# monoamine11231/Example-GUI-OpenCL-Raytracer

Hardware: AMD Instinct MI355X
Metric: Mrays/s at 1920x1080 depth 4, aggregate over n_gpus; rays = path segments + shadow rays as the reference casts them (value_traced: only those the kernel really traces) (higher is better)
Workload: dtype f32; 1 GPU; C2: scenes/render.map (regenerated), camera raypng.c:17-21, 1920x1080, depth 4, 2 soft-shadow samples, 4x256^2 textures + 4096x3072 skybox (procedural); frame=1920x1080, arithmetic=fast

## Files before the change

example_gui_opencl_raytracer_amd/csrc/hip_wrap.cpp:

```cpp
#include <hip/hip_runtime.h>

#include <algorithm>
#include <cstdarg>
#include <cstdint>
#include <cstdio>
#include <cstdlib>
#include <cmath>
#include <cstring>
#include <string>
#include <vector>

#include "../../include/hip_wrap_ext.h"
#include "png_codec.h"
#include "scene_prep.h"
#include "whitted_params.h"

extern "C" hipError_t wt_fast_launch_trace(const whitted_params*, int, unsigned, size_t, hipStream_t);
extern "C" hipError_t wt_fast_launch_raygen(const raygen_params*, hipStream_t);
extern "C" hipError_t wt_strict_launch_trace(const whitted_params*, int, unsigned, size_t, hipStream_t);
extern "C" hipError_t wt_strict_launch_raygen(const raygen_params*, hipStream_t);
extern "C" hipError_t wt_fast_launch_unit(int, const float*, float*, unsigned, unsigned, unsigned, unsigned, hipStream_t);
extern "C" hipError_t wt_strict_launch_unit(int, const float*, float*, unsigned, unsigned, unsigned, unsigned, hipStream_t);
extern "C" hipError_t wt_fast_launch_unit_scene(const whitted_params*, int, int, const float*, float*, unsigned, unsigned, unsigned, size_t, hipStream_t);
extern "C" hipError_t wt_strict_launch_unit_scene(const whitted_params*, int, int, const float*, float*, unsigned, unsigned, unsigned, size_t, hipStream_t);
// ... 77 lines not shown
    ArgValue values[__MAX_BUFFERS];
};

struct TimingEntry { hipEvent_t start, stop; cl_uint kernel; };

struct Impl {
    int device = 0;
    hipStream_t own_stream = nullptr;
    hipStream_t stream = nullptr;
    std::vector<Kernel> kernels;
    std::vector<Buffer*> live;
    int depth = 15;
    int strict = 0;
    int fuse = 1;
    int async = 0;
    int variant = 0;
    int last_trace_flags = -1;
    int counting = 0;
    float through = 0.8f;
    int stamps = 0;
    uint64_t id_offset = 0;
    uint32_t band_stride = 1, band_phase = 0;
    int supersample = 1;
    float* debug_rgb = nullptr;
    std::vector<clw_sample_camera> cams;
    float aperture = 0.0f, focus = 1.0f;
    std::vector<clw_sample_camera> cams_used;
    float* d_cams = nullptr;
    wt_cam_table cams_dev{}; bool cams_dev_valid = false;
    hipEvent_t cams_fence = nullptr; bool cams_fence_pending = false, cams_in_flight = false;
    const Buffer *prep_s = nullptr, *prep_p = nullptr, *prep_l = nullptr;
    uint32_t prep_ns = 0, prep_np = 0, prep_nl = 0;
    float* d_geom = nullptr; size_t geom_f4 = 0;
    float* d_ptex = nullptr;
    bool have_lpt = false;
    uint64_t scene_generation = 0;
    uint32_t *d_grid_start = nullptr, *d_grid_items = nullptr, *d_grid_box = nullptr;
    float* d_grid_geom = nullptr;
    wprep_grid grid{}; bool grid_ok = false, grid_pair = false; int use_grid = 1;
    unsigned long long* d_counters = nullptr;
    int sched = 1;
    struct Sched {
        unsigned* cost[2] = {nullptr, nullptr}; unsigned* order[2] = {nullptr, nullptr};
        hipEvent_t built[2] = {nullptr, nullptr};
        bool have[2] = {false, false};
        int wr = 0;
        hipEvent_t traced = nullptr;
        uint32_t w = 0, rows = 0, cap = 0;
        int ss = 1;
        wt_cam_table sig_cams{}; bool sig_has_cams = false;
        RaygenArgs sig{}; int sig_depth = 0; uint64_t sig_scene = 0; bool sig_valid = false; int sig_age = 0, newest = 0; uint64_t frame = 0, newest_frame = 0;
        void reset() { have[0] = have[1] = false; sig_valid = false; newest = 0; }
        void free_all() {
            for (int i = 0; i < 2; i++) {
                if (cost[i]) (void)hipFree(cost[i]);
                if (order[i]) (void)hipFree(order[i]);
                if (built[i]) (void)hipEventDestroy(built[i]);
                cost[i] = order[i] = nullptr; built[i] = nullptr;
            }
            if (traced) { (void)hipEventDestroy(traced); traced = nullptr; }
            reset();
        }
    };
    hipStream_t sched_stream = nullptr;
    static constexpr int MAX_CHUNKS = 4;
    Sched scheds[1 + MAX_CHUNKS];
// ... 173 lines not shown
float env_float(const char* name, float dflt) {
    const char* s = getenv(name);
    if (!s || !*s) return dflt;
    char* end = nullptr;
    const float v = strtof(s, &end);
    return (end == s || *end) ? NAN : v;
}

void xorshift_jump_matrices(uint32_t steps, uint32_t out[7][32]) {
    auto apply = [](const uint32_t* A, uint32_t x) { uint32_t r = 0; for (int b = 0; b < 32; b++) if ((x >> b) & 1u) r ^= A[b]; return r; };
    auto mul = [&](const uint32_t* A, const uint32_t* B, uint32_t* C) { uint32_t t[32]; for (int b = 0; b < 32; b++) t[b] = apply(A, B[b]); memcpy(C, t, sizeof t); };
    uint32_t T[32], R[32], Bp[32];
    for (int b = 0; b < 32; b++) { uint32_t x = 1u << b; x ^= x << 13; x ^= x >> 17; x ^= x << 5; T[b] = x; R[b] = 1u << b; }
    memcpy(Bp, T, sizeof T);
    for (uint32_t e = steps; e; e >>= 1) { if (e & 1u) mul(Bp, R, R); mul(Bp, Bp, Bp); }
    memcpy(out[0], R, sizeof R);
    for (int i = 1; i < 7; i++) mul(out[i - 1], out[i - 1], out[i]);
}

void prepare_scene(Impl* I, Buffer* s, uint32_t ns, Buffer* p, uint32_t np, Buffer* l, uint32_t nl) {
    if (I->d_geom && I->prep_s == s && I->prep_p == p && I->prep_l == l && I->prep_ns == ns &&
        I->prep_np == np && I->prep_nl == nl)
        return;
    std::vector<uint8_t> ts, tp, tl;
    const uint8_t* hs = host_view(I, s, 96 * (size_t)ns, ts);
    const uint8_t* hp = host_view(I, p, 96 * (size_t)np, tp);
    const uint8_t* hl = host_view(I, l, 48 * (size_t)nl, tl);
    const size_t base_f4 = wprep_geom_f4(ns, np, nl), lpt_f4 = wprep_lpt_f4(np, nl);
    size_t f4 = base_f4 + lpt_f4;
    std::vector<float> geom(4 * (f4 ? f4 : 1)), ptex(8 * (size_t)(np ? np : 1));
    wprep_build(hs, ns, hp, np, hl, nl, geom.data(), ptex.data());
    wprep_build_lpt(hp, np, hl, nl, geom.data() + 4 * base_f4);
    I->have_lpt = lpt_f4 != 0;
    {
        uint32_t jm[7][32];
        xorshift_jump_matrices(4u * nl, jm);
        if (!I->d_tpt_jump) HIP_OK(hipMalloc((void**)&I->d_tpt_jump, sizeof jm), "Couldn't allocate device memory");
        HIP_OK(hipMemcpy(I->d_tpt_jump, jm, sizeof jm, hipMemcpyHostToDevice), "Couldn't transfer the data from host to the device");
    }
    if (I->d_geom) { (void)hipFree(I->d_geom); I->d_geom = nullptr; }
    if (I->d_ptex) { (void)hipFree(I->d_ptex); I->d_ptex = nullptr; }
    HIP_OK(hipMalloc((void**)&I->d_geom, geom.size() * 4), "Couldn't allocate device memory");
    HIP_OK(hipMalloc((void**)&I->d_ptex, ptex.size() * 4), "Couldn't allocate device memory");
    HIP_OK(hipMemcpy(I->d_geom, geom.data(), geom.size() * 4, hipMemcpyHostToDevice), "Couldn't transfer the data from host to the device");
    HIP_OK(hipMemcpy(I->d_ptex, ptex.data(), ptex.size() * 4, hipMemcpyHostToDevice), "Couldn't transfer the data from host to the device");
    for (uint32_t** q : {&I->d_grid_start, &I->d_grid_items, &I->d_grid_box}) { if (*q) { (void)hipFree(*q); *q = nullptr; } }
    if (I->d_grid_geom) { (void)hipFree(I->d_grid_geom); I->d_grid_geom = nullptr; }
    I->grid_ok = false;
    if (ns > (uint32_t)env_int("CLWRAP_GRID_MIN", (int)GRID_MIN_SPHERES)) {
        const char* dens = getenv("CLWRAP_GRID_DENSITY");
        float maxr = 0.0f;
        for (uint32_t l = 0; l < nl; l++) { float r; memcpy(&r, hl + 48 * (size_t)l + 16, 4); r = fabsf(r); if (!(r <= maxr)) maxr = r; }
        const float density = dens ? (float)atof(dens) : 1.6f;
        size_t pairs = 0;
        I->grid_pair = false;
        if (env_int("CLWRAP_GRID_PAIR", 1) && nl > 0 && maxr > 0.0f && std::isfinite(maxr)) {
            pairs = wprep_grid_plan(hs, ns, density, maxr, &I->grid);
            I->grid_pair = maxr <= 0.3f * std::min(I->grid.cell[0], std::min(I->grid.cell[1], I->grid.cell[2])) && pairs <= GRID_MAX_PAIRS;
        }
        if (!I->grid_pair) pairs = wprep_grid_plan(hs, ns, density, 0.0f, &I->grid);
        if (pairs <= GRID_MAX_PAIRS) {
            std::vector<uint32_t> st((size_t)I->grid.ncells + 1), it(pairs ? pairs : 1), bx(2 * (size_t)ns);
            wprep_grid_fill(hs, ns, &I->grid, st.data(), it.data(), bx.data());
            HIP_OK(hipMalloc((void**)&I->d_grid_start, st.size() * 4), "Couldn't allocate device memory");
            HIP_OK(hipMalloc((void**)&I->d_grid_items, it.size() * 4), "Couldn't allocate device memory");
            HIP_OK(hipMalloc((void**)&I->d_grid_box, bx.size() * 4), "Couldn't allocate device memory");
// ... 48 lines not shown
        dyn_lds = I->geom_f4 * 16;
    }
}

struct Strip { uint32_t row0, rows; int slot; };

void run_raytracer(cl_wrap* w, Impl* I, cl_uint kid, size_t array_size, const Strip* strip = nullptr) {
    Kernel& k = I->kernels[kid];
    Buffer* rays = nullptr;
    if (is_registered(w, kid, 0)) rays = (Buffer*)w->buffers[kid][0];
    else {
        const ArgValue& v = need_value(k, 0, sizeof(cl_mem), sizeof(cl_mem));
        void* h; memcpy(&h, v.bytes, sizeof h);
        rays = lookup_handle(I, h);
        if (!rays) die("Couldn't run the kernel");
    }
    uint32_t total; memcpy(&total, need_value(k, 7, 4, 4).bytes, 4);
    Buffer* out = buffer_arg(w, kid, 10);

    uint64_t rounded = ((uint64_t)array_size + BLOCK - 1) / BLOCK * BLOCK;
    uint64_t n64 = rounded < total ? rounded : total;
    ensure_allocated(I, out);
    if (n64 > out->size / 4) n64 = out->size / 4;
    if (n64 == 0) return;
    if (n64 > 0xFFFFFFFFull) die("Couldn't run the kernel");

    whitted_params P{};
    int flags = 0;
    size_t dyn_lds = 0;
    bind_scene(w, I, kid, P, flags, dyn_lds);
    P.n_items = (uint32_t)n64;
    P.depth = I->depth;
    P.untrimmed = (I->variant & 16384) ? 1u : 0u;
    P.out = (uint32_t*)out->dptr;
    P.out_rgb = I->debug_rgb;
    P.diag = (I->variant & 512) ? (env_int("CLWRAP_TIMELINE_EDGES", 0) ? 255u + (uint32_t)env_int("CLWRAP_TIMELINE_EDGES", 0) : 1u + (uint32_t)env_int("CLWRAP_TIMELINE_SHIFT", 0)) : 0u;

    const int ss = I->supersample;
    if (I->aperture > 0.0f && ss == 1) die("A lens needs samples: aperture %g with supersampling factor 1 (clw_ext_set_supersample / CLWRAP_SUPERSAMPLE)", (double)I->aperture);
    if (!I->cams.empty() && (ss == 1 || I->cams.size() != (size_t)(ss * ss)))
        die("Sample cameras: the table holds %u cameras, but supersampling factor %d %s", (unsigned)I->cams.size(), ss,
            ss == 1 ? "takes none (set a factor of 2, 4 or 8)" : (ss == 2 ? "needs 4" : (ss == 4 ? "needs 16" : "needs 64")));
    bool have_cams = false;
    wt_cam_table cam_table;
    I->cams_used.clear();
    const bool fused = I->fuse && rays->gen_valid && !rays->exposed;
    RaygenArgs g{};
    if (fused) {
        g = rays->gen;
        if (strip) {
            g.id_offset += (uint64_t)strip->row0 * g.width;
            g.n_items = strip->rows * g.width;
            P.n_items = g.n_items;
            P.out = (uint32_t*)out->dptr + (size_t)strip->row0 * g.width;
        }
        memcpy(P.corner, g.corner, 12); memcpy(P.origin, g.origin, 12);
        memcpy(P.up, g.up, 12); memcpy(P.right, g.right, 12);
        P.w_factor = g.w_factor; P.h_factor = g.h_factor; P.width = g.width; P.height = g.height;
        P.id_offset = g.id_offset;
        P.band_stride = g.band_stride; P.band_phase = g.band_phase;
        if (P.n_items > g.n_items) P.n_items = g.n_items;
        if (P.n_items == 0) return;
        P.tiled = (g.id_offset % g.width == 0 || g.band_stride > 1) && (P.n_items % g.width == 0) && !(I->variant & 2);
        if (ss > 1) {
            if (g.band_stride > 1) die("Supersampling does not support interleaved row bands");
            if (I->variant & 2) die("Supersampling does not support linear work-item ids (variant 2)");
// ... 84 lines not shown
            split = tail_wanted && !(flags & F_GRID) && I->split_min_quota != 0u && !(I->variant & 4096) && split_max_lg != 0u;
            if (split) { per_share_cap = per_share + SPLIT_EXTRA_PER_SHARE; grid = 8 * per_share_cap; }
            P.cost_sum = (tail_wanted && !(flags & F_GRID)) ? 1u : 0u;
            if (S.w != P.width || S.rows != P.rows || S.cap != per_share_cap || S.ss != ss || !S.cost[0]) {
                S.free_all();
                for (int i = 0; i < 2; i++) {
                    HIP_OK(hipMalloc((void**)&S.cost[i], (size_t)trows * tpr * 4), "Couldn't allocate device memory");
                    HIP_OK(hipMalloc((void**)&S.order[i], (size_t)grid * 4), "Couldn't allocate device memory");
                    HIP_OK(hipEventCreateWithFlags(&S.built[i], hipEventDisableTiming), "Couldn't create a timing event");
                }
                HIP_OK(hipEventCreateWithFlags(&S.traced, hipEventDisableTiming), "Couldn't create a timing event");
                S.w = P.width; S.rows = P.rows; S.cap = per_share_cap; S.ss = ss; S.wr = 0;
            }
            const int wr = S.wr;
            P.tile_cost = S.cost[wr];
            int rd = S.have[S.newest] ? S.newest : -1;
            if (rd >= 0 && S.frame - S.newest_frame <= 1 && S.have[rd ^ 1]) rd ^= 1;
            S.frame++;
            if (S.have[wr]) HIP_OK(hipStreamWaitEvent(I->stream, S.built[wr], 0), "Couldn't run the kernel");
            if (rd >= 0 && rd != wr) HIP_OK(hipStreamWaitEvent(I->stream, S.built[rd], 0), "Couldn't run the kernel");
            P.tile_order = rd >= 0 ? S.order[rd] : nullptr;
            sched_rebuild = !S.sig_valid || !same_raygen(g, S.sig) || S.sig_depth != I->depth || S.sig_scene != I->scene_generation ||
                            S.sig_has_cams != have_cams || (have_cams && memcmp(&S.sig_cams, &cam_table, sizeof cam_table));
            if (P.cost_sum) HIP_OK(hipMemsetAsync(S.cost[wr], 0, (size_t)trows * tpr * 4, I->stream), "Couldn't run the kernel");
            if (sched_rebuild) { S.sig_has_cams = have_cams; if (have_cams) S.sig_cams = cam_table; S.sig = g; S.sig_depth = I->depth; S.sig_scene = I->scene_generation; S.sig_valid = true; S.sig_age = 0; }
            else if ((flags & F_GRID) && S.sig_age < 2) sched_rebuild = true;
            if (S.sig_age < 255) S.sig_age++;
        }
    }
    if ((flags & F_DEEP) && !(flags & F_COUNT) && !(I->variant & 2048)) flags |= I->depth <= 8 ? F_D8 : (I->depth <= 16 ? F_D16 : 0);
    if (!I->strict && flags == F_GEOM_LDS && P.ns >= 1u && P.ns <= SHAPE_MAX_SPHERES && P.np <= SHAPE_MAX_PLANES && P.nl == SHAPE_LIGHTS &&
        (P.np == 0u || P.lpt) && !(I->variant & 8192))
        flags |= F_SHAPE | (int)(P.ns << 9 | P.np << 12 | P.nl << 14);
    if (P.ss_lg) flags |= F_SS;
    I->last_trace_flags = flags;
    if (tail_wanted) {
        const uint64_t nslots = tpt_nslots, slice = tpt_slice, cap = tpt_cap;
        if (cap >= TPT_MIN_CAP) {
            const size_t need = (size_t)slice * 4u * nslots;
            if (I->tpt_pool_bytes != need) {
                finish(I);
                if (I->d_tpt_pool) (void)hipFree(I->d_tpt_pool);
                if (I->d_tpt_flags) (void)hipFree(I->d_tpt_flags);
                I->d_tpt_pool = nullptr; I->d_tpt_flags = nullptr; I->tpt_pool_bytes = 0;
                if (hipMalloc((void**)&I->d_tpt_pool, need) == hipSuccess && hipMalloc((void**)&I->d_tpt_flags, nslots * 4u) == hipSuccess) {
                    HIP_OK(hipMemset(I->d_tpt_flags, 0, nslots * 4u), "Couldn't allocate device memory");
                    I->tpt_pool_bytes = need;
                } else {
                    (void)hipGetLastError();
                    if (I->d_tpt_pool) (void)hipFree(I->d_tpt_pool);
                    I->d_tpt_pool = nullptr;
                }
            }
            if (I->tpt_pool_bytes) {
                P.tpt_pool = I->d_tpt_pool; P.tpt_flags = I->d_tpt_flags; P.tpt_slice_words = (uint32_t)slice; P.tpt_cap = (uint32_t)cap;
                P.tpt_slots = TPT_SLOTS_PER_XCC; P.tpt_jump = I->d_tpt_jump;
                P.tpt_max = std::min(I->tpt_max, 64u); P.tpt_min = I->tpt_min;
            }
        }
    }
    LaunchTimer t(I, kid);
    hipError_t e = I->strict ? wt_strict_launch_trace(&P, flags, grid, dyn_lds, I->stream)
                             : wt_fast_launch_trace(&P, flags, grid, dyn_lds, I->stream);
    if (e != hipSuccess) die("Couldn't run the kernel");
    t.done();
    if (P.tile_cost) {
// ... 487 lines not shown
```

example_gui_opencl_raytracer_amd/csrc/scene_prep.c:

```c
#include "scene_prep.h"
#include <string.h>
#include <math.h>
#include <stdlib.h>

#define INV_PI_F 0.31830988618379067154f

static float ldf(const uint8_t* p, size_t off) { float f; memcpy(&f, p + off, 4); return f; }
static uint32_t ldu(const uint8_t* p, size_t off) { uint32_t u; memcpy(&u, p + off, 4); return u; }

static void cross(const float a[3], const float b[3], float out[3]) {
    out[0] = a[1] * b[2] - a[2] * b[1];
    out[1] = a[2] * b[0] - a[0] * b[2];
    out[2] = a[0] * b[1] - a[1] * b[0];
}

size_t wprep_geom_f4(uint32_t ns, uint32_t np, uint32_t nl) { return (size_t)ns + 2 * (size_t)np + 2 * (size_t)nl; }

void wprep_build(const uint8_t* spheres, uint32_t ns, const uint8_t* planes, uint32_t np,
                 const uint8_t* lights, uint32_t nl, float* geom, float* ptex) {
    float* g = geom;
    for (uint32_t i = 0; i < ns; i++, g += 4) {
        const uint8_t* s = spheres + 96 * (size_t)i;
        float r = ldf(s, 16);
        float r2 = r * r;
// ... 8 lines not shown
    for (uint32_t i = 0; i < np; i++, g += 8) {
        const uint8_t* p = planes + 96 * (size_t)i;
        float n[3] = {ldf(p, 0), ldf(p, 4), ldf(p, 8)};
        int32_t texture_id = (int32_t)ldu(p, 32 + 48);
        float scale = ldf(p, 32 + 52);
        g[0] = n[0]; g[1] = n[1]; g[2] = n[2]; g[3] = texture_id >= 0 ? 1.0f : 0.0f;
        g[4] = ldf(p, 16); g[5] = ldf(p, 20); g[6] = ldf(p, 24); g[7] = 0.0f;

        static const float axes[3][3] = {{1.0f, 0.0f, 0.0f}, {0.0f, 1.0f, 0.0f}, {0.0f, 0.0f, 1.0f}};
        float b0[3] = {0, 0, 0}, b1[3] = {0, 0, 0};
        for (int a = 0; a < 3; a++) {
            float cr[3];
            cross(axes[a], n, cr);
            float sum = 1.0f * cr[0] + 1.0f * cr[1] + 1.0f * cr[2];
            if (sum == 0.0f) continue;
            memcpy(b0, cr, sizeof b0);
            cross(n, cr, b1);
            break;
        }
        float* t = ptex + 8 * (size_t)i;
        t[0] = b0[0]; t[1] = b0[1]; t[2] = b0[2]; t[3] = scale;
        t[4] = b1[0]; t[5] = b1[1]; t[6] = b1[2];
        memcpy(&t[7], &texture_id, 4);
    }
    for (uint32_t i = 0; i < nl; i++, g += 8) {
        const uint8_t* l = lights + 48 * (size_t)i;
        float r = ldf(l, 16), intensity = ldf(l, 20);
        g[0] = ldf(l, 0); g[1] = ldf(l, 4); g[2] = ldf(l, 8); g[3] = r * r;
        for (int k = 0; k < 3; k++) {
            float c = ldf(l, 32 + 4 * (size_t)k);
            g[4 + k] = (c * intensity) * INV_PI_F;
        }
        g[7] = r;
    }
}

size_t wprep_lpt_f4(uint32_t np, uint32_t nl) {
    size_t n = (size_t)((nl + 2) / 3) * np;
    return n <= 64 ? n : 0;
}
void wprep_build_lpt(const uint8_t* planes, uint32_t np, const uint8_t* lights, uint32_t nl, float* out) {
    if (!wprep_lpt_f4(np, nl)) return;
    for (uint32_t c = 0; c < (nl + 2) / 3; c++)
        for (uint32_t p = 0; p < np; p++) {
            const uint8_t* pl = planes + 96 * (size_t)p;
            double n[3] = {ldf(pl, 0), ldf(pl, 4), ldf(pl, 8)}, p0[3] = {ldf(pl, 16), ldf(pl, 20), ldf(pl, 24)};
            double nn = sqrt(n[0] * n[0] + n[1] * n[1] + n[2] * n[2]);
            float* o = out + 4 * ((size_t)c * np + p);
            for (int k = 0; k < 3; k++) {
                o[k] = 0.0f;
                uint32_t l = 3 * c + (uint32_t)k;
                if (l >= nl || !(nn > 0.0) || !isfinite(nn)) continue;
                const uint8_t* li = lights + 48 * (size_t)l;
                double L[3] = {ldf(li, 0), ldf(li, 4), ldf(li, 8)}, r = fabs((double)ldf(li, 16));
                double sd = ((L[0] - p0[0]) * n[0] + (L[1] - p0[1]) * n[1] + (L[2] - p0[2]) * n[2]) / nn;
                double mag = fabs(L[0]) + fabs(L[1]) + fabs(L[2]) + fabs(p0[0]) + fabs(p0[1]) + fabs(p0[2]);
                double mu = fabs(sd) - r * (1.0 + 1e-5) - 1e-5 * mag - 1e-30;
                if (isfinite(mu) && mu > 0.0) o[k] = (float)(sd > 0 ? mu : -mu) * (1.0f - 1e-6f);
            }
            o[3] = (nn > 0.0 && isfinite(nn)) ? (float)(1.0 / nn) : 0.0f;
        }
}

static void sphere_cells(const uint8_t* s, const wprep_grid* g, int lo[3], int hi[3]) {
    float r = ldf(s, 16);
    for (int a = 0; a < 3; a++) {
// ... 93 lines not shown
```

example_gui_opencl_raytracer_amd/csrc/scene_prep.h:

```cpp
#ifndef WHITTED_SCENE_PREP_H
#define WHITTED_SCENE_PREP_H
#include <stdint.h>
#include <stddef.h>
#ifdef __cplusplus
extern "C" {
#endif
size_t wprep_geom_f4(uint32_t ns, uint32_t np, uint32_t nl);
void wprep_build(const uint8_t* spheres, uint32_t ns, const uint8_t* planes, uint32_t np,
                 const uint8_t* lights, uint32_t nl, float* geom, float* ptex);

size_t wprep_lpt_f4(uint32_t np, uint32_t nl);
void wprep_build_lpt(const uint8_t* planes, uint32_t np, const uint8_t* lights, uint32_t nl, float* out);

typedef struct {
    float gmin[3], inv[3], cell[3];
    int32_t res[3];
    uint32_t ncells;
    float reg_pad;
} wprep_grid;
size_t wprep_grid_plan(const uint8_t* spheres, uint32_t ns, float density, float reg_pad, wprep_grid* g);
void wprep_grid_fill(const uint8_t* spheres, uint32_t ns, const wprep_grid* g, uint32_t* start, uint32_t* items,
                     uint32_t* box);
#ifdef __cplusplus
}
#endif
#endif
```

example_gui_opencl_raytracer_amd/csrc/whitted_hit.inc:

```
            cost++;
            if (COUNT) {
                c_iter++;
                unsigned long long live = __builtin_amdgcn_ballot_w64(true);
                if (lane == (unsigned)__builtin_ctzll(live)) c_witer += 64u;
            }
            const rayq r = UNIT_CT ? wt_rayq<true>(o, d) : wt_rayq<false>(o, d, P.unit_dirs != 0u);

            if (COUNT) c_probe++;
            bool lit = false;
            float tl = INFINITY;
            f3 lcol = mk3(0, 0, 0);
            auto probe_chunk = [&](auto nc, const unsigned base) {
                constexpr int N = decltype(nc)::value;
                float4 l0[N]; float bq[N], Dq[N]; bool ok[N]; bool any = false;
#pragma unroll
                for (int k = 0; k < N; k++) l0[k] = wt_geom<GEOM_LDS>(P, sg, g_lgt + 2 * (base + k));
#pragma unroll
                for (int k = 0; k < N; k++) {
                    const sph_pre pre = wt_sphere_pre(r.o, l0[k]);
                    ok[k] = wt_sphere_disc(pre, r.d, r.a4, bq[k], Dq[k]);
                    any |= ok[k];
                }
                if (__builtin_amdgcn_ballot_w64(any)) {
#pragma unroll
                    for (int k = 0; k < N; k++) {
                        float t;
                        const bool hit = wt_sphere_root(bq[k], Dq[k], r.a2, t) && ok[k];
                        if (hit && !(t >= tl)) {
                            float4 l1 = wt_geom<GEOM_LDS>(P, sg, g_lgt + 2 * (base + k) + 1);
                            tl = t;
                            f3 hp = wt_madd3(d, t, o);
                            float dist = wt_sqrt(dot3(o - hp, o - hp));
                            lcol = mk3(l1.x, l1.y, l1.z) * (1 / dist * dist);
                            lit = true;
                        }
                    }
                }
            };
            for (unsigned base = 0; base < SH::nl(P); base += 4u) {
                const unsigned left = SH::nl(P) - base;
                if (left >= 4u) probe_chunk(wt_int<4>{}, base);
                else if (left == 3u) probe_chunk(wt_int<3>{}, base);
                else if (left == 2u) probe_chunk(wt_int<2>{}, base);
                else probe_chunk(wt_int<1>{}, base);
            }
            if (__builtin_amdgcn_ballot_w64(lit)) {
                if (lit) {
                    if (GRID) {
                        if (wt_grid_occluded(P, r, tl)) lit = false;
                    }
                    for (unsigned i = 0; !GRID && i < SH::ns(P); i++) {
                        float4 s = wt_geom<GEOM_LDS>(P, sg, i);
                        float t;
                        bool hit = wt_sphere(r, s, t);
                        if (hit && t <= tl && !(__float_as_uint(s.w) >> 31)) lit = false;
                    }
                    for (unsigned i = 0; i < SH::np(P); i++) {
                        float4 n = wt_geom<GEOM_LDS>(P, sg, g_pln + 2 * i);
                        float4 p0 = wt_geom<GEOM_LDS>(P, sg, g_pln + 2 * i + 1);
                        float t;
                        bool hit = wt_plane(r, n, p0, t);
                        if (hit && t <= tl) lit = false;
                    }
                }
            }
            WT_STAMP(WT_ST_PROBE);
            if (lit) {
                WT_HIT_COLOUR(lcol);
                ended = true;
            } else {
                if (COUNT) c_seg++;
                float tbest = INFINITY;
                int best = -1;
                if (GRID) {
                    best = wt_grid_nearest(P, r, tbest);
                } else {
                    for (unsigned base = 0; base < SH::ns(P); base += 4u) {
                        float4 s4[4]; float bq[4], Dq[4]; bool ok[4]; bool any = false;
#pragma unroll
                        for (int k = 0; k < 4; k++) s4[k] = wt_geom<GEOM_LDS>(P, sg, min(base + k, SH::ns(P) - 1u));
#pragma unroll
                        for (int k = 0; k < 4; k++) {
                            const sph_pre pre = wt_sphere_pre(r.o, s4[k]);
                            ok[k] = wt_sphere_disc(pre, r.d, r.a4, bq[k], Dq[k]) && (base + k < SH::ns(P));
                            any |= ok[k];
                        }
                        if (__builtin_amdgcn_ballot_w64(any)) {
#pragma unroll
                            for (int k = 0; k < 4; k++) {
                                if (__builtin_amdgcn_ballot_w64(ok[k]) == 0) continue;
                                float t;
                                const bool hit = wt_sphere_root(bq[k], Dq[k], r.a2, t) && ok[k];
                                if (hit && !(t >= tbest)) { tbest = t; best = (int)(base + k); }
                            }
                        }
                    }
                }
                for (unsigned i = 0; i < SH::np(P); i++) {
                    float4 n = wt_geom<GEOM_LDS>(P, sg, g_pln + 2 * i);
                    float4 p0 = wt_geom<GEOM_LDS>(P, sg, g_pln + 2 * i + 1);
                    float t;
                    bool hit = wt_plane(r, n, p0, t);
                    if (hit && !(t >= tbest)) { tbest = t; best = (int)(SH::ns(P) + i); }
                }
                WT_STAMP(WT_ST_NEAREST);
                if (best < 0) {
                    if (COUNT) c_sky++;
                    WT_HIT_COLOUR(wt_texel_rgb(wt_skybox_fetch(P, d)));
                    ended = true;
                } else {
                    ip = wt_madd3(d, tbest, o);
                    prim = (unsigned)best;
                    textured = false;
                    if ((unsigned)best < SH::ns(P)) {
                        float4 s = wt_geom<GEOM_LDS>(P, sg, (unsigned)best);
                        nrm = wt_normalize(ip - mk3(s.x, s.y, s.z));
                    } else {
                        unsigned pi = (unsigned)best - SH::ns(P);
                        float4 n = wt_geom<GEOM_LDS>(P, sg, g_pln + 2 * pi);
                        nrm = mk3(n.x, n.y, n.z);
                        if (n.w != 0.0f) {
                            if (COUNT) c_tex++;
                            texpx = wt_plane_texel_fetch(P, pi, ip);
                            textured = true;
                        }
                    }
                    wt_mat_set_b(m, wt_mat_f4(P, prim, 1u, SH::ns(P)));
                    {
                        const float4 a_ = wt_mat_f4(P, prim, 0u, SH::ns(P));
                        m.rgb = mk3(a_.x, a_.y, a_.z);
                        wt_mat_set_c(m, wt_mat_f4(P, prim, 2u, SH::ns(P)));
                    }
                    ip = wt_madd3(nrm, WT_EPSILON, ip);
                    cost += 3u;
                    {
// ... 9 lines not shown
```

example_gui_opencl_raytracer_amd/csrc/whitted_params.h:

```cpp
#ifndef WHITTED_PARAMS_H
#define WHITTED_PARAMS_H
#include <stdint.h>

#define CLW_MAX_DEPTH 32
#define CLW_NUM_COUNTERS 32
#define CLW_STAMP_SHARDS 1024

typedef struct {
    float corner[3], origin[3], up[3], right[3];
    float w_factor, h_factor;
    uint32_t width, height;
    uint64_t id_offset;
    uint32_t n_items;
    uint32_t tiled;
    uint32_t rows;
    uint32_t row_offset;
    uint32_t band_stride, band_phase;
    const uint32_t* tile_order;
    uint32_t* tile_cost;
    uint32_t* tpt_pool;
    uint32_t* tpt_flags;
    const uint32_t* tpt_jump;
    uint32_t tpt_slice_words, tpt_cap, tpt_slots, tpt_max, tpt_min;
    uint32_t tpt_clock;
    uint32_t cost_sum;
    int32_t depth;
    uint32_t untrimmed;
    const float* geom;
    const float* ptex;
    const uint8_t* spheres_raw;
    const uint8_t* planes_raw;
    uint32_t ns, np, nl;
    float through;
    uint32_t geom_f4;
    uint32_t unit_dirs;
    uint32_t lpt;
    uint32_t vis;
    uint32_t diag;
    const uint32_t* grid_start;
    const uint32_t* grid_items;
    const uint32_t* grid_box;
    const float* grid_geom;
    float grid_min[3], grid_inv[3], grid_cell[3];
    uint32_t grid_pair;
    int32_t grid_res[3];
    const uint32_t* tex; int32_t tex_w, tex_h, tex_layers;
    const uint32_t* sky; int32_t sky_w, sky_h;
    const float* rays;
    uint32_t* out;
    float* out_rgb;
    unsigned long long* counters;
    uint32_t ss_lg;
    const float* ss_cams;
} whitted_params;

#define WT_CAM_TABLE_FLOATS (64 * 12)
typedef struct { float v[WT_CAM_TABLE_FLOATS]; } wt_cam_table;

typedef struct {
    float corner[3], origin[3], up[3], right[3];
    float w_factor, h_factor;
    uint32_t width, height;
    uint64_t id_offset;
    uint32_t n_items;
    uint32_t band_stride, band_phase;
    float* rays;
} raygen_params;

#endif
```

example_gui_opencl_raytracer_amd/csrc/whitted_pop.inc:

```
        while (active && (ended || depth >= D)) {
            if (sp == 0) { active = false; break; }
            sp--;
            float rec[WT_REC];
            if (SCRL == 0 || sp < LDSL) {
#pragma unroll
                for (int w = 0; w < WT_REC; w++) rec[w] = s_stk[(sp * WT_REC + w) * WT_BLOCK + tid];
            } else {
#pragma unroll
                for (int w = 0; w < WT_REC; w++) rec[w] = deep[(sp - LDSL) * WT_REC + w];
            }
            o = mk3(rec[0], rec[1], rec[2]);
            d = mk3(rec[3], rec[4], rec[5]);
            rgb = mk3(rec[6], rec[7], rec[8]) + rgb;
            depth = __float_as_int(rec[9]);
            n1 = rec[10];
            f = rec[11];
            ended = false;
        }
```

example_gui_opencl_raytracer_amd/csrc/whitted_terms.inc:

```
#undef WT_HIT_COLOUR
#undef WT_HIT_AMBIENT
#undef WT_SHADE_ADD
#undef WT_BOUNCE_PUSH
#undef WT_BOUNCE_LAST
#define WT_HIT_COLOUR(c) rgb = wt_madd3((c), f, rgb)
#define WT_HIT_AMBIENT(cf, a) rgb = wt_madd3((cf), (a), rgb)
#define WT_SHADE_ADD(li, l1, soft, dl, spec, diff) rgb = wt_light_add(rgb, (l1), (soft), (dl), (spec), (diff), ks, kd)
#define WT_BOUNCE_PUSH(rec) do { \
        if (SCRL == 0 || sp < LDSL) { _Pragma("unroll") for (int w_ = 0; w_ < WT_REC; w_++) s_stk[(sp * WT_REC + w_) * WT_BLOCK + tid] = (rec)[w_]; } \
        else { _Pragma("unroll") for (int w_ = 0; w_ < WT_REC; w_++) deep[(sp - LDSL) * WT_REC + w_] = (rec)[w_]; } \
        sp++; rgb = mk3(0, 0, 0); } while (0)
#define WT_BOUNCE_LAST (depth >= D && !P.untrimmed)
```

example_gui_opencl_raytracer_amd/csrc/whitted_trace.inc:

```

#ifndef WT_STRICT
#error "WT_STRICT must be defined (0: fast, 1: strict)"
#endif

#define WT_EPSILON 0.001f
#define WT_THROUGH 0.8f
#define WT_DEFAULT_N 1.0f
#define WT_SOFT 2
#ifndef WT_LDS_LEVELS
#if WT_STRICT
#define WT_LDS_LEVELS 3
#else
#define WT_LDS_LEVELS 2
#endif
#endif
#ifndef WT_LDS_LEVELS_DEEP
#define WT_LDS_LEVELS_DEEP 3
#endif
#ifndef WT_LDS_LEVELS_DEEP_OCC
#define WT_LDS_LEVELS_DEEP_OCC 1
#endif
#ifndef WT_MIN_WAVES
#define WT_MIN_WAVES (WT_STRICT ? 2 : 3)
#endif
// ... 177 lines not shown
    x ^= x << 13;
    x ^= x >> 17;
    x ^= x << 5;
    s = x;
    return (float)x * 9.31322574615478515625e-10f;
}

struct rayq {
    f3 o, d;
    float a4;
    float a2;
};
template <bool UNIT>
__device__ __forceinline__ rayq wt_rayq(f3 o, f3 d, bool unit_rt = false) {
    rayq r; r.o = o; r.d = d;
#if !WT_STRICT
    if (UNIT || unit_rt) { r.a4 = 1.0f; r.a2 = 1.0f; return r; }
#endif
    float a = dot3(d, d);
    r.a4 = a;
#if WT_STRICT
    r.a2 = a;
#else
    r.a2 = __builtin_amdgcn_rcpf(a);
#endif
    return r;
}

struct sph_pre { f3 v2; float c; };
__device__ __forceinline__ sph_pre wt_sphere_pre(f3 o, float4 s) {
    sph_pre p;
    p.v2 = o - mk3(s.x, s.y, s.z);
    p.c = dot3(p.v2, p.v2) - fabsf(s.w);
    return p;
}
__device__ __forceinline__ bool wt_sphere_disc(const sph_pre& p, f3 d, float a4, float& b, float& D) {
    b = dot3(p.v2, d);
    D = wt_fma(b, b, -(a4 * p.c));
    return !(D < 0);
}
__device__ __forceinline__ bool wt_sphere_root(float b, float D, float a2, float& t) {
    float sD = wt_sqrt(D);
#if WT_STRICT
    float t0 = (-b - sD) / a2;
    float t2 = (t0 < 0) ? (-b + sD) / a2 : t0;
#else
    float t0 = (-b - sD) * a2;
    float t2 = (t0 < 0) ? (-b + sD) * a2 : t0;
#endif
    t = t2;
    return !(t2 <= 0);
}
__device__ __forceinline__ bool wt_sphere_dir(const sph_pre& p, f3 d, float a4, float a2, float& t) {
    float b, D;
    bool ok = wt_sphere_disc(p, d, a4, b, D);
    return wt_sphere_root(b, D, a2, t) && ok;
}
__device__ __forceinline__ bool wt_sphere(const rayq& r, float4 s, float& t) {
    const sph_pre p = wt_sphere_pre(r.o, s);
    float b, D;
    const bool ok = wt_sphere_disc(p, r.d, r.a4, b, D);
    bool hit = false;
    t = 0.0f;
    if (__builtin_amdgcn_ballot_w64(ok)) hit = wt_sphere_root(b, D, r.a2, t) && ok;
    return hit;
}
// ... 889 lines not shown
            if (P.tiled || P.band_stride > 1u) d = wt_primary_dir_xy(P.corner, P.right, P.up, P.w_factor, P.h_factor, x, gy);
            else d = wt_primary_dir(P.corner, P.right, P.up, P.w_factor, P.h_factor, (unsigned)gid, P.width);
            o = mk3(P.origin[0], P.origin[1], P.origin[2]);
        }
    }
    float n1 = WT_DEFAULT_N, f = 1.0f;
    int sp = 0;
    unsigned rng = (unsigned)gid;
    const int D = P.depth;
    bool active = valid && depth < D;

    unsigned c_seg = 0, c_shadow = 0, c_probe = 0, c_sky = 0, c_tex = 0, c_push = 0, c_iter = 0, c_witer = 0;
    unsigned c_traced = 0;
    unsigned c_known = 0, c_visbad = 0;
    unsigned c_tptrun = 0, c_tptfail = 0, c_tptnodes = 0;

    typedef wt_shape<FLAGS> SH;
    const unsigned g_pln = SH::ns(P), g_lgt = SH::ns(P) + 2 * SH::np(P);

    const unsigned long long t_begin = ((GRID || WT_COST_LIFETIME) && P.tile_cost) ? __builtin_amdgcn_s_memtime() : 0ull;
#if WT_TIMELINE
    const unsigned long long tl_begin = __builtin_amdgcn_s_memrealtime();
    unsigned long long tl_end = tl_begin;
#endif
    unsigned cost = 0;
#ifndef WT_LCH
#define WT_LCH 3
#endif
    constexpr int LCH = WT_LCH, NR = LCH * WT_SOFT;

    constexpr bool TPT = DEEP && !wt_cfg<FLAGS>::occ;
    unsigned tpt_thresh = (TPT && P.tpt_cap != 0u) ? (part_lg != 0u ? 64u : P.tpt_max) : 0u;
    WT_STAMP(WT_ST_PROLOG);
    for (;;) {
    while ((unsigned)__builtin_popcountll(__builtin_amdgcn_ballot_w64(active)) > tpt_thresh) {
        if (active) {
            WT_STAMP(WT_ST_LOOP);
            bool ended = false, shade = false;
            f3 ip, nrm, view;
            mat_t m;
            float ks, kd;
            unsigned prim, texpx;
            bool textured;
#include "whitted_hit.inc"
            WT_STAMP(WT_ST_RESOLVE);
            if (shade) {
#include "whitted_shade.inc"
#include "whitted_bounce.inc"
            WT_STAMP(WT_ST_BOUNCE);
            }
#include "whitted_pop.inc"
            WT_STAMP(WT_ST_POP);
        }
    }
    if (!TPT || __builtin_amdgcn_ballot_w64(active) == 0) break;
    {
        bool tpt_done = false;
#include "whitted_tpt.inc"
        if (tpt_done) break;
        tpt_thresh = 0u;
    }
    }
    if (P.tiled && P.tile_cost) {
        unsigned c = cost;
        if (GRID || WT_COST_LIFETIME) c = (unsigned)min((__builtin_amdgcn_s_memtime() - t_begin) >> 8, 0xFFFFFFFFull);
        else if (P.untrimmed) {
// ... 330 lines not shown
```

Measured before the change: 350,100 Mrays/s.

## Peel primary ray iteration using host-precomputed origin-dependent sphere and plane terms

The first trace iteration is peeled out for shaped fast kernels. All primary rays share the camera origin, so the per-sphere offset and constant term and the per-plane numerator are computed once on the host. They are passed in the kernel params, and the peeled hit test reads them instead of recomputing them from geometry. This trims ALU and geometry loads on the primary segment, at the cost of more code size, a larger params struct and possible register pressure. A variant bit disables the peel.

Measured after the change: 350,200 Mrays/s (median of 2 runs). No clear change (+0.0%).

```diff
diff --git a/example_gui_opencl_raytracer_amd/csrc/hip_wrap.cpp b/example_gui_opencl_raytracer_amd/csrc/hip_wrap.cpp
--- a/example_gui_opencl_raytracer_amd/csrc/hip_wrap.cpp
+++ b/example_gui_opencl_raytracer_amd/csrc/hip_wrap.cpp
@@ -133,6 +133,7 @@
     const Buffer *prep_s = nullptr, *prep_p = nullptr, *prep_l = nullptr;
     uint32_t prep_ns = 0, prep_np = 0, prep_nl = 0;
     float* d_geom = nullptr; size_t geom_f4 = 0;
+    std::vector<float> h_geom;
     float* d_ptex = nullptr;
     bool have_lpt = false;
     uint64_t scene_generation = 0;
@@ -372,6 +373,7 @@
     wprep_build(hs, ns, hp, np, hl, nl, geom.data(), ptex.data());
     wprep_build_lpt(hp, np, hl, nl, geom.data() + 4 * base_f4);
     I->have_lpt = lpt_f4 != 0;
+    I->h_geom = geom;
     {
         uint32_t jm[7][32];
         xorshift_jump_matrices(4u * nl, jm);
@@ -486,6 +488,7 @@
     P.n_items = (uint32_t)n64;
     P.depth = I->depth;
     P.untrimmed = (I->variant & 16384) ? 1u : 0u;
+    P.unpeeled = (I->variant & 32768) ? 1u : 0u;
     P.out = (uint32_t*)out->dptr;
     P.out_rgb = I->debug_rgb;
     P.diag = (I->variant & 512) ? (env_int("CLWRAP_TIMELINE_EDGES", 0) ? 255u + (uint32_t)env_int("CLWRAP_TIMELINE_EDGES", 0) : 1u + (uint32_t)env_int("CLWRAP_TIMELINE_SHIFT", 0)) : 0u;
@@ -636,6 +639,11 @@
     if (!I->strict && flags == F_GEOM_LDS && P.ns >= 1u && P.ns <= SHAPE_MAX_SPHERES && P.np <= SHAPE_MAX_PLANES && P.nl == SHAPE_LIGHTS &&
         (P.np == 0u || P.lpt) && !(I->variant & 8192))
         flags |= F_SHAPE | (int)(P.ns << 9 | P.np << 12 | P.nl << 14);
+    if (flags & F_SHAPE) {
+        static_assert(SHAPE_MAX_SPHERES == WT_PRIM_MAX_SPHERES && SHAPE_MAX_PLANES == WT_PRIM_MAX_PLANES && SHAPE_LIGHTS == WT_PRIM_MAX_LIGHTS,
+                      "the primary-segment table is sized for the shaped kernels' counts");
+        wprep_primary_terms(I->h_geom.data(), P.ns, P.np, P.nl, P.origin, 0, &P.prim_sph[0][0], &P.prim_lgt[0][0], P.prim_pln);
+    }
     if (P.ss_lg) flags |= F_SS;
     I->last_trace_flags = flags;
     if (tail_wanted) {
diff --git a/example_gui_opencl_raytracer_amd/csrc/scene_prep.c b/example_gui_opencl_raytracer_amd/csrc/scene_prep.c
--- a/example_gui_opencl_raytracer_amd/csrc/scene_prep.c
+++ b/example_gui_opencl_raytracer_amd/csrc/scene_prep.c
@@ -64,6 +64,29 @@
             g[4 + k] = (c * intensity) * INV_PI_F;
         }
         g[7] = r;
+    }
+}
+
+static float prim_dot3(const float a[3], const float b[3], int strict) {
+    if (strict) return a[0] * b[0] + a[1] * b[1] + a[2] * b[2];
+    return fmaf(a[2], b[2], fmaf(a[1], b[1], a[0] * b[0]));
+}
+static void prim_sphere_pre(const float* s, const float o[3], int strict, float out[4]) {
+    const float v[3] = {o[0] - s[0], o[1] - s[1], o[2] - s[2]};
+    out[0] = v[0]; out[1] = v[1]; out[2] = v[2];
+    out[3] = prim_dot3(v, v, strict) - fabsf(s[3]);
+}
+void wprep_primary_terms(const float* geom, uint32_t ns, uint32_t np, uint32_t nl, const float origin[3], int strict,
+                         float* sph, float* lgt, float* pln) {
+    const float* planes = geom + 4 * (size_t)ns;
+    const float* lights = planes + 8 * (size_t)np;
+    for (uint32_t i = 0; i < ns; i++) prim_sphere_pre(geom + 4 * (size_t)i, origin, strict, sph + 4 * (size_t)i);
+    for (uint32_t i = 0; i < nl; i++) prim_sphere_pre(lights + 8 * (size_t)i, origin, strict, lgt + 4 * (size_t)i);
+    for (uint32_t i = 0; i < np; i++) {
+        const float* n = planes + 8 * (size_t)i;
+        const float* p0 = n + 4;
+        const float w[3] = {p0[0] - origin[0], p0[1] - origin[1], p0[2] - origin[2]};
+        pln[i] = prim_dot3(w, n, strict);
     }
 }
 
diff --git a/example_gui_opencl_raytracer_amd/csrc/scene_prep.h b/example_gui_opencl_raytracer_amd/csrc/scene_prep.h
--- a/example_gui_opencl_raytracer_amd/csrc/scene_prep.h
+++ b/example_gui_opencl_raytracer_amd/csrc/scene_prep.h
@@ -12,6 +12,9 @@
 size_t wprep_lpt_f4(uint32_t np, uint32_t nl);
 void wprep_build_lpt(const uint8_t* planes, uint32_t np, const uint8_t* lights, uint32_t nl, float* out);
 
+void wprep_primary_terms(const float* geom, uint32_t ns, uint32_t np, uint32_t nl, const float origin[3], int strict,
+                         float* sph, float* lgt, float* pln);
+
 typedef struct {
     float gmin[3], inv[3], cell[3];
     int32_t res[3];
diff --git a/example_gui_opencl_raytracer_amd/csrc/whitted_hit.inc b/example_gui_opencl_raytracer_amd/csrc/whitted_hit.inc
--- a/example_gui_opencl_raytracer_amd/csrc/whitted_hit.inc
+++ b/example_gui_opencl_raytracer_amd/csrc/whitted_hit.inc
@@ -17,7 +17,7 @@
                 for (int k = 0; k < N; k++) l0[k] = wt_geom<GEOM_LDS>(P, sg, g_lgt + 2 * (base + k));
 #pragma unroll
                 for (int k = 0; k < N; k++) {
-                    const sph_pre pre = wt_sphere_pre(r.o, l0[k]);
+                    const sph_pre pre = WT_HIT_LIGHT_PRE(r.o, l0[k], base + k);
                     ok[k] = wt_sphere_disc(pre, r.d, r.a4, bq[k], Dq[k]);
                     any |= ok[k];
                 }
@@ -81,7 +81,7 @@
                         for (int k = 0; k < 4; k++) s4[k] = wt_geom<GEOM_LDS>(P, sg, min(base + k, SH::ns(P) - 1u));
 #pragma unroll
                         for (int k = 0; k < 4; k++) {
-                            const sph_pre pre = wt_sphere_pre(r.o, s4[k]);
+                            const sph_pre pre = WT_HIT_SPHERE_PRE(r.o, s4[k], min(base + k, SH::ns(P) - 1u));
                             ok[k] = wt_sphere_disc(pre, r.d, r.a4, bq[k], Dq[k]) && (base + k < SH::ns(P));
                             any |= ok[k];
                         }
@@ -100,7 +100,7 @@
                     float4 n = wt_geom<GEOM_LDS>(P, sg, g_pln + 2 * i);
                     float4 p0 = wt_geom<GEOM_LDS>(P, sg, g_pln + 2 * i + 1);
                     float t;
-                    bool hit = wt_plane(r, n, p0, t);
+                    bool hit = wt_plane_dir(WT_HIT_PLANE_NUM(r.o, n, p0, i), n, r.d, t);
                     if (hit && !(t >= tbest)) { tbest = t; best = (int)(SH::ns(P) + i); }
                 }
                 WT_STAMP(WT_ST_NEAREST);
diff --git a/example_gui_opencl_raytracer_amd/csrc/whitted_params.h b/example_gui_opencl_raytracer_amd/csrc/whitted_params.h
--- a/example_gui_opencl_raytracer_amd/csrc/whitted_params.h
+++ b/example_gui_opencl_raytracer_amd/csrc/whitted_params.h
@@ -5,6 +5,10 @@
 #define CLW_MAX_DEPTH 32
 #define CLW_NUM_COUNTERS 32
 #define CLW_STAMP_SHARDS 1024
+
+#define WT_PRIM_MAX_SPHERES 4
+#define WT_PRIM_MAX_PLANES 2
+#define WT_PRIM_MAX_LIGHTS 3
 
 typedef struct {
     float corner[3], origin[3], up[3], right[3];
@@ -52,6 +56,8 @@
     unsigned long long* counters;
     uint32_t ss_lg;
     const float* ss_cams;
+    float prim_sph[WT_PRIM_MAX_SPHERES][4], prim_lgt[WT_PRIM_MAX_LIGHTS][4], prim_pln[WT_PRIM_MAX_PLANES];
+    uint32_t unpeeled;
 } whitted_params;
 
 #define WT_CAM_TABLE_FLOATS (64 * 12)
diff --git a/example_gui_opencl_raytracer_amd/csrc/whitted_pop.inc b/example_gui_opencl_raytracer_amd/csrc/whitted_pop.inc
--- a/example_gui_opencl_raytracer_amd/csrc/whitted_pop.inc
+++ b/example_gui_opencl_raytracer_amd/csrc/whitted_pop.inc
@@ -1,4 +1,5 @@
-        while (active && (ended || depth >= D)) {
+        if (WT_POP_ROOT) { if (active && (ended || depth >= D)) active = false; }
+        else while (active && (ended || depth >= D)) {
             if (sp == 0) { active = false; break; }
             sp--;
             float rec[WT_REC];
diff --git a/example_gui_opencl_raytracer_amd/csrc/whitted_terms.inc b/example_gui_opencl_raytracer_amd/csrc/whitted_terms.inc
--- a/example_gui_opencl_raytracer_amd/csrc/whitted_terms.inc
+++ b/example_gui_opencl_raytracer_amd/csrc/whitted_terms.inc
@@ -3,6 +3,10 @@
 #undef WT_SHADE_ADD
 #undef WT_BOUNCE_PUSH
 #undef WT_BOUNCE_LAST
+#undef WT_HIT_LIGHT_PRE
+#undef WT_HIT_SPHERE_PRE
+#undef WT_HIT_PLANE_NUM
+#undef WT_POP_ROOT
 #define WT_HIT_COLOUR(c) rgb = wt_madd3((c), f, rgb)
 #define WT_HIT_AMBIENT(cf, a) rgb = wt_madd3((cf), (a), rgb)
 #define WT_SHADE_ADD(li, l1, soft, dl, spec, diff) rgb = wt_light_add(rgb, (l1), (soft), (dl), (spec), (diff), ks, kd)
@@ -11,3 +15,7 @@
         else { _Pragma("unroll") for (int w_ = 0; w_ < WT_REC; w_++) deep[(sp - LDSL) * WT_REC + w_] = (rec)[w_]; } \
         sp++; rgb = mk3(0, 0, 0); } while (0)
 #define WT_BOUNCE_LAST (depth >= D && !P.untrimmed)
+#define WT_HIT_LIGHT_PRE(o, l0, i) wt_sphere_pre((o), (l0))
+#define WT_HIT_SPHERE_PRE(o, s, i) wt_sphere_pre((o), (s))
+#define WT_HIT_PLANE_NUM(o, n, p0, i) wt_plane_pre((o), (n), (p0))
+#define WT_POP_ROOT false
diff --git a/example_gui_opencl_raytracer_amd/csrc/whitted_trace.inc b/example_gui_opencl_raytracer_amd/csrc/whitted_trace.inc
--- a/example_gui_opencl_raytracer_amd/csrc/whitted_trace.inc
+++ b/example_gui_opencl_raytracer_amd/csrc/whitted_trace.inc
@@ -233,6 +233,12 @@
     sph_pre p;
     p.v2 = o - mk3(s.x, s.y, s.z);
     p.c = dot3(p.v2, p.v2) - fabsf(s.w);
+    return p;
+}
+__device__ __forceinline__ sph_pre wt_prim_pre(const float* q) {
+    sph_pre p;
+    p.v2 = mk3(q[0], q[1], q[2]);
+    p.c = q[3];
     return p;
 }
 __device__ __forceinline__ bool wt_sphere_disc(const sph_pre& p, f3 d, float a4, float& b, float& D) {
@@ -1188,6 +1194,39 @@
     constexpr bool TPT = DEEP && !wt_cfg<FLAGS>::occ;
     unsigned tpt_thresh = (TPT && P.tpt_cap != 0u) ? (part_lg != 0u ? 64u : P.tpt_max) : 0u;
     WT_STAMP(WT_ST_PROLOG);
+    constexpr bool PEEL = !WT_STRICT && SH::on && !FROM_RAYS && !SS && !DEEP && !GRID;
+    if constexpr (PEEL) {
+    if (!P.unpeeled) {
+        if (active) {
+            WT_STAMP(WT_ST_LOOP);
+            o = mk3(P.origin[0], P.origin[1], P.origin[2]);
+            bool ended = false, shade = false;
+            f3 ip, nrm, view;
+            mat_t m;
+            float ks, kd;
+            unsigned prim, texpx;
+            bool textured;
+#undef WT_HIT_LIGHT_PRE
+#undef WT_HIT_SPHERE_PRE
+#undef WT_HIT_PLANE_NUM
+#undef WT_POP_ROOT
+#define WT_HIT_LIGHT_PRE(o, l0, i) wt_prim_pre(P.prim_lgt[i])
+#define WT_HIT_SPHERE_PRE(o, s, i) wt_prim_pre(P.prim_sph[i])
+#define WT_HIT_PLANE_NUM(o, n, p0, i) (P.prim_pln[i])
+#define WT_POP_ROOT true
+#include "whitted_hit.inc"
+            WT_STAMP(WT_ST_RESOLVE);
+            if (shade) {
+#include "whitted_shade.inc"
+#include "whitted_bounce.inc"
+            WT_STAMP(WT_ST_BOUNCE);
+            }
+#include "whitted_pop.inc"
+            WT_STAMP(WT_ST_POP);
+#include "whitted_terms.inc"
+        }
+    }
+    }
     for (;;) {
     while ((unsigned)__builtin_popcountll(__builtin_amdgcn_ballot_w64(active)) > tpt_thresh) {
         if (active) {
```
